# joyecnu/STTODE

Measured on AMD Instinct MI355X. Metric: predicted-trajectories/sec (20-sample best-of-K), higher is better.
Workload: dtype f32

## Files before the change

sttode_amd/csrc/chain32.hip:

```cpp
#include "chain.hpp"
#include "latency_bodies.hpp"
#include "frontend_body.hpp"
#include "api_util.hpp"
#include "../../include/sttode_hip.h"
#include <cstdlib>
#include <cstddef>

#ifdef C32_DIAG_TRACE
__shared__ long long g_tr_ph[4];
#define C32_TRACE_BEGIN() long long _tr_t0 = 0, _tr_c0 = 0; if (threadIdx.x == 0 && A.dbg) { _tr_t0 = __builtin_amdgcn_s_memrealtime(); _tr_c0 = __builtin_amdgcn_s_memtime(); }
#define C32_TRACE_END(kind) do { if (threadIdx.x == 0 && A.dbg) { \
        const long long _t1 = __builtin_amdgcn_s_memrealtime(); unsigned _hw, _xcc; \
        asm volatile("s_getreg_b32 %0, hwreg(HW_REG_HW_ID)" : "=s"(_hw)); asm volatile("s_getreg_b32 %0, hwreg(HW_REG_XCC_ID)" : "=s"(_xcc)); \
        const unsigned long long _r = atomicAdd((unsigned long long*)A.dbg, 1ull); if ((long long)_r >= A.dbg[1]) break;  \
        long long* _p = A.dbg + 8 + _r * 12; _p[0] = A.trace_tag; _p[1] = blockIdx.x; _p[2] = (kind); _p[3] = _tr_t0; _p[4] = _t1; _p[5] = _hw; _p[6] = _xcc; \
        _p[8] = g_tr_ph[0]; _p[9] = g_tr_ph[1]; _p[10] = g_tr_ph[2]; _p[7] = __builtin_amdgcn_s_memtime() - _tr_c0; _p[11] = g_tr_ph[3]; } } while (0)
#define C32_TRACE_PHASE(i) do { if (threadIdx.x == 0) g_tr_ph[i] = __builtin_amdgcn_s_memrealtime(); } while (0)
#else
#define C32_TRACE_PHASE(i) do { } while (0)
#define C32_TRACE_BEGIN() do { } while (0)
#define C32_TRACE_END(kind) do { } while (0)
#endif

#include "role_body.hpp"

typedef float f32x16 __attribute__((ext_vector_type(16)));

#ifdef C32_DIAG_NOGATES
#define C32_SIG(x) ((x) * 1e-3f)
#define C32_TANH(x) ((x) * 1e-3f)
#else
#define C32_SIG(x) sigmoid_prescaled(x)
#define C32_TANH(x) tanh_prescaled(x)
#endif

#define C32_TILE 256
#define C32_CMAX 3
#define C32_RING (2 * C32_CMAX * C32_TILE)
#define C32_SLOT 256

struct Role32Args {
    const f32x4* pool; const int2* prog; int prog_len; const float* consts;
    const float* enc_in; const int* last;
    const float* g_in; const float* attn; int ld_attn;
    const float* xpad; int ldx;
    float* pf; float* state0; float* A0x; float* A0y; float* A1y;
    int n, Tp, kte, nwg;
    float ode_time;
    int prio;
    int* counter;
    float* zgen; unsigned zkey0, zkey1; int K;
    const float* past; const int* scene_ptr; int S; float* scene_orig; int* agent_scene;
    float* enc_in_w; float* xpad_w; float* cur_w; float* orig_w; int* last_w;
    float* m_ade; float* m_fde;
};

struct ChainArgs {
    const float* A0x; const float* A0y; const float* A1y;
    const f32x4* pool;
    const int2* prog; int prog_len;
    const float* consts;
    const float* z;
    const float* xpad; int ldx;
    const float* cur; const float* orig;
    float* pred;
    float* park;
    int* counter;
    int ncols, K, Tp, Tf2;
    int persistent;
    const float* m_gt; float* m_ade; float* m_fde; float m_scale;
    int nworkers;
    long long* dbg;
    int trace_tag;
    int xcd_map;
    RoleArgs R;
    Role32Args R32;
};

template <int NY> struct C32Const {
    static constexpr int b2x = 0, b3x = 256, b2y = 288, b3y = 544, gb = 544 + 32 * NY, cb = gb + 384, b2m = cb + 32,
                         b3m = b2m + 256, total = b3m + 32 * NY;
};

__device__ __forceinline__ f32x16 splat16(float v) {
    f32x16 r;
#pragma unroll
    for (int e = 0; e < 16; ++e) r[e] = v;
    return r;
}
__device__ __forceinline__ f32x16 relu16(f32x16 v) {
#pragma unroll
    for (int e = 0; e < 16; ++e) v[e] = fmaxf(v[e], 0.f);
    return v;
}
__device__ __forceinline__ f32x16 ldrows(const float* p, int h) {
    f32x16 r;
#pragma unroll
    for (int a = 0; a < 4; ++a) {
        const f32x4 v = ld4(p + 8 * a + 4 * h);
        r[4 * a + 0] = v[0]; r[4 * a + 1] = v[1]; r[4 * a + 2] = v[2]; r[4 * a + 3] = v[3];
    }
    return r;
}

typedef const __attribute__((address_space(4))) int KProg;

template <int BUF, bool GEN, bool DYN = false>
struct ChainStreamT {
    static constexpr int kBuf = BUF;
    static constexpr int kPieces = (BUF / 64 + 3) / 4, kPairs = (kPieces + 1) / 2;
    const char* pool; KProg* prog; f32x4* ring;
    unsigned ring_addr, loff;
    unsigned qoff, qend;
    int par, lane, wave;
    int2 ld_v, ld_w;
    bool fetched;
    int cnt;
    const char* nsrc[kPairs]; unsigned nm0[kPairs]; int ncnt, npc;
#ifdef C32_DIAG_STAMPS
    long long t_bar, gap_cyc, gap_n, gap_cal;
#endif
    __device__ __forceinline__ int2 entry_at(unsigned off) const {
        const KProg* e = reinterpret_cast<const KProg*>(reinterpret_cast<const __attribute__((address_space(4))) char*>(prog) + off);
        return make_int2(e[0], e[1]);
    }
    __device__ __forceinline__ unsigned next_off(unsigned off) const { return off + 8 >= qend ? 0u : off + 8; }
    __device__ __forceinline__ void stage(int2 ev, int buf) {
        ncnt = __builtin_amdgcn_readfirstlane(ev.y);
        npc = GEN ? (ncnt - wave + 3) >> 2 : ncnt;
        const size_t src = (size_t)(unsigned)__builtin_amdgcn_readfirstlane(ev.x) * (GEN ? 16u : C32_TILE * 16u) + (unsigned)wave * 1024u;
        const unsigned dst = __builtin_amdgcn_readfirstlane(ring_addr + (unsigned)buf * (BUF * 16) + (unsigned)wave * 1024u);
#pragma unroll
        for (int k = 0; k < kPairs; ++k) {
            nsrc[k] = pool + (src + 4096u * (2 * k + 1));
            nm0[k] = dst + 4096u * (2 * k + 1);
            asm volatile("" : "+s"(nsrc[k]), "+s"(nm0[k]));
        }
        asm volatile("" : "+s"(npc));
    }
    __device__ __forceinline__ void issue(int N) {
#ifndef C32_DIAG_NODMA
#pragma unroll
        for (int k = 0; k < kPairs; ++k) {
            if (N > 0 ? 2 * k < N : 2 * k < npc) {
                glds16_sv<-4096>(nsrc[k], loff, nm0[k] - 4096u);
                if (2 * k + 1 < kPieces && (N > 0 ? 2 * k + 1 < N : 2 * k + 1 < npc)) glds16_m0<0>(nsrc[k], loff);
            }
        }
#endif
    }
    __device__ __forceinline__ void init(const f32x4* pool_, const int2* prog_, int len_, f32x4* ring_) {
        pool = reinterpret_cast<const char*>(pool_); prog = (KProg*)prog_; ring = ring_;
        ring_addr = __builtin_amdgcn_readfirstlane(lds_addr(ring_));
        lane = threadIdx.x & 63;
        loff = (unsigned)lane * 16;
        wave = __builtin_amdgcn_readfirstlane(threadIdx.x >> 6);
        par = 0;
        qend = (unsigned)len_ * 8u;
        const int2 e0 = entry_at(0);
        stage(e0, 0);
        issue(0);
        cnt = e0.y;
        qoff = next_off(0);
        stage(entry_at(qoff), 1);
        qoff = next_off(qoff);
        fetched = false;
#ifdef C32_DIAG_STAMPS
        gap_cyc = 0; gap_n = 0;
        const long long c0 = __builtin_amdgcn_s_memtime();
        asm volatile("s_waitcnt lgkmcnt(0)" ::: "memory");
        gap_cal = __builtin_amdgcn_s_memtime() - c0;
        t_bar = 0;
#endif
    }
    __device__ __forceinline__ void fetch() { ld_v = entry_at(qoff); qoff = next_off(qoff); fetched = true; }
    __device__ __forceinline__ void fetch_more() { ld_w = entry_at(qoff); qoff = next_off(qoff); }
    __device__ __forceinline__ void take_prefetched() { ld_v = ld_w; fetched = true; }
    __device__ __forceinline__ void stamp_gap() {
#ifdef C32_DIAG_STAMPS
        asm volatile("s_waitcnt lgkmcnt(0)" ::: "memory");
        const long long c1 = __builtin_amdgcn_s_memtime();
        asm volatile("s_waitcnt lgkmcnt(0)" ::: "memory");
        if (t_bar) { gap_cyc += c1 - t_bar; ++gap_n; }
#endif
    }
    __device__ __forceinline__ void begin(int N = 0) {
        __builtin_amdgcn_sched_barrier(0);
#ifdef C32_DIAG_CHECK
        if (!GEN && N > 0 && ncnt != N) __builtin_trap();
#endif
        cnt = ncnt;
        issue(GEN || DYN ? 0 : N);
        stamp_gap();
        __builtin_amdgcn_sched_barrier(0);
    }
    __device__ __forceinline__ const f32x4* cur() const { return ring + par * BUF + lane; }
    __device__ __forceinline__ void end(bool has_entry = false) {
        __builtin_amdgcn_sched_barrier(0);
#ifdef C32_DIAG_CHECK
        if (has_entry && !fetched) __builtin_trap();
#endif
        if (!has_entry && !fetched) fetch();
        stage(ld_v, par);
        __builtin_amdgcn_sched_barrier(0);
#ifndef C32_DIAG_NOBARRIER
        asm volatile("s_waitcnt vmcnt(0)" ::: "memory");
        __syncthreads();
#endif
#ifdef C32_DIAG_STAMPS
        t_bar = __builtin_amdgcn_s_memtime();
        asm volatile("s_waitcnt lgkmcnt(0)" ::: "memory");
#endif
        par ^= 1;
        fetched = false;
        __builtin_amdgcn_sched_barrier(0);
    }
};
typedef ChainStreamT<C32_CMAX * C32_TILE, false> ChainStream;

__device__ __forceinline__ void tile_mma(f32x16& acc, const f32x4* __restrict__ t, const f32x16& B) {
#pragma unroll
    for (int g = 0; g < 4; ++g) {
        const f32x4 a = t[g * 64];
#pragma unroll
        for (int r = 0; r < 4; ++r) acc = __builtin_amdgcn_mfma_f32_32x32x2f32(a[r], B[4 * g + r], acc, 0, 0, 0);
    }
}

__device__ __forceinline__ void gather_rows(const void* base, unsigned voff, unsigned slot_addr) {
    glds16_sv<0>(base, voff, slot_addr);
    glds16_sv<32>(base, voff, slot_addr + 1024);
    glds16_sv<64>(base, voff, slot_addr + 2048);
    glds16_sv<96>(base, voff, slot_addr + 3072);
}
__device__ __forceinline__ unsigned row_off(int row, int width, int h) { return (unsigned)row * (unsigned)(width * 4) + (unsigned)h * 16; }

struct Frag { f32x4 a[4]; };
__device__ __forceinline__ void ldfrag(Frag& f, const f32x4* __restrict__ t) {
#pragma unroll
    for (int g = 0; g < 4; ++g) f.a[g] = t[g * 64];
}
__device__ __forceinline__ void tile_mma2(f32x16& acc, const Frag& cur, const f32x16& B, Frag& nxt, const f32x4* __restrict__ tn) {
#pragma unroll
    for (int g = 0; g < 4; ++g) {
        if (g == 2 && tn) {
            ldfrag(nxt, tn);
            __builtin_amdgcn_sched_barrier(0);
        }
#pragma unroll
        for (int r = 0; r < 4; ++r) acc = __builtin_amdgcn_mfma_f32_32x32x2f32(cur.a[g][r], B[4 * g + r], acc, 0, 0, 0);
    }
}

template <class ST>
__device__ __forceinline__ void tile_mma2f(ST& st, f32x16& acc, const Frag& cur, const f32x16& B, Frag& nxt, const f32x4* __restrict__ tn, int nf = 1) {
#pragma unroll
    for (int g = 0; g < 4; ++g) {
        if (g == 2) {
            __builtin_amdgcn_sched_barrier(0);
            if (nf >= 1) st.fetch();
            if (nf >= 2) st.fetch_more();
            if (tn) ldfrag(nxt, tn);
            __builtin_amdgcn_sched_barrier(0);
        }
#pragma unroll
        for (int r = 0; r < 4; ++r) acc = __builtin_amdgcn_mfma_f32_32x32x2f32(cur.a[g][r], B[4 * g + r], acc, 0, 0, 0);
    }
}

template <int KH, class ST>
__device__ __forceinline__ void mlp_l12(ST& st, const f32x4* slot, const f32x4* zslot, const f32x16* Bh, const float* tab, unsigned aoff,
                                        const float* tab_next, unsigned aoff_next, f32x16 (&acc2)[8], int lane) {
    const unsigned slot_addr = __builtin_amdgcn_readfirstlane(lds_addr(slot));
    constexpr int KT1 = 1 + KH;
    static_assert((KT1 + 8) % 3 == 0, "hidden tile must be a whole number of chunks");
#pragma unroll
    for (int R = 0; R < 8; ++R) acc2[R] = splat16(0.f);
#pragma unroll 1
    for (int ht = 0; ht < 16; ++ht) {
        f32x16 h1, zb;
#pragma unroll
        for (int a = 0; a < 4; ++a) {
            const f32x4 v = slot[a * 64 + lane];
            h1[4 * a + 0] = v[0]; h1[4 * a + 1] = v[1]; h1[4 * a + 2] = v[2]; h1[4 * a + 3] = v[3];
        }
#pragma unroll
        for (int a = 0; a < 4; ++a) {
            const f32x4 v = zslot[a * 64 + lane];
            zb[4 * a + 0] = v[0]; zb[4 * a + 1] = v[1]; zb[4 * a + 2] = v[2]; zb[4 * a + 3] = v[3];
        }
        asm volatile("s_waitcnt lgkmcnt(0)" ::: "memory");
        __builtin_amdgcn_sched_barrier(0);
        const bool nl = ht + 1 < 16;
        const void* nb = nl ? (const void*)(reinterpret_cast<const char*>(tab) + 128 * (ht + 1)) : (const void*)tab_next;
        const unsigned no = nl ? aoff : aoff_next;
        Frag fr[2];
#pragma unroll
        for (int i = 0; i < KT1 + 8; ++i) {
            if (i % 3 == 0) {
                if (i > 0) st.end();
                ldfrag(fr[i & 1], st.cur());
                st.begin(3);
                if (i == 0) {
#ifndef C32_DIAG_NOGATHER
                    gather_rows(nb, no, slot_addr);
#endif
                    __builtin_amdgcn_sched_barrier(0);
                }
            }
            const f32x4* tn = (i % 3 < 2) ? st.cur() + (i % 3 + 1) * C32_TILE : nullptr;
            if (i == 0) {
                tile_mma2f(st, h1, fr[i & 1], zb, fr[(i + 1) & 1], tn);
            } else if (i < KT1) {
                if (i % 3 == 0) tile_mma2f(st, h1, fr[i & 1], Bh[i - 1], fr[(i + 1) & 1], tn);
                else tile_mma2(h1, fr[i & 1], Bh[i - 1], fr[(i + 1) & 1], tn);
            } else {
                if (i == KT1) h1 = relu16(h1);
                if (i % 3 == 0) tile_mma2f(st, acc2[i - KT1], fr[i & 1], h1, fr[(i + 1) & 1], tn);
                else tile_mma2(acc2[i - KT1], fr[i & 1], h1, fr[(i + 1) & 1], tn);
            }
        }
        st.end();
    }
}

template <int NO, int NEXT = 0, class ST>
__device__ __forceinline__ void mlp_l3(ST& st, f32x16 (&acc2)[8], const float* __restrict__ b2, const float* __restrict__ b3,
                                       f32x16 (&out)[NO], int h) {
#pragma unroll
    for (int R = 0; R < 8; ++R) {
        STT_FENCE();
        const f32x16 b = ldrows(b2 + 32 * R, h);
        acc2[R] = relu16(acc2[R] + b);
        asm volatile("" : "+v"(acc2[R]));
    }
    STT_FENCE();
#pragma unroll
    for (int o = 0; o < NO; ++o) out[o] = ldrows(b3 + 32 * o, h);
    Frag fr[2];
#pragma unroll
    for (int i = 0; i < 8 * NO; ++i) {
        if (i % 3 == 0) {
            if (i > 0) st.end();
            ldfrag(fr[i & 1], st.cur());
            const int left = 8 * NO - (i + 3);
            st.begin(left >= 3 ? 3 : left > 0 ? left : NEXT);
        }
        const f32x4* tn = (i % 3 < 2 && i + 1 < 8 * NO) ? st.cur() + (i % 3 + 1) * C32_TILE : nullptr;
        if (i % 3 == 0) tile_mma2f(st, out[i / 8], fr[i & 1], acc2[i % 8], fr[(i + 1) & 1], tn);
        else tile_mma2(out[i / 8], fr[i & 1], acc2[i % 8], fr[(i + 1) & 1], tn);
    }
    st.end();
}

typedef __bf16 bf16x8 __attribute__((ext_vector_type(8)));
typedef __bf16 bf16x2 __attribute__((ext_vector_type(2)));
typedef float f32x2v __attribute__((ext_vector_type(2)));
typedef unsigned u32x4v __attribute__((ext_vector_type(4)));
#define C32_TILE_B3 384
#define C32_BUF_B3 (C32_CMAX * C32_TILE_B3)
struct B3 { bf16x8 p[3][2]; };
__device__ __forceinline__ float bf_lo(unsigned u) { return __uint_as_float(u << 16); }
__device__ __forceinline__ float bf_hi(unsigned u) { return __uint_as_float(u & 0xffff0000u); }
__device__ __forceinline__ void split3(const f32x16& x, B3& o) {
#pragma unroll
    for (int kb = 0; kb < 2; ++kb) {
        unsigned hi[4], mi[4], lo[4];
#pragma unroll
        for (int q = 0; q < 4; ++q) {
            const float x0 = x[8 * kb + 2 * q], x1 = x[8 * kb + 2 * q + 1];
            const f32x2v v = {x0, x1};
            hi[q] = __builtin_bit_cast(unsigned, __builtin_convertvector(v, bf16x2));
            const float r0 = x0 - bf_lo(hi[q]), r1 = x1 - bf_hi(hi[q]);
            const f32x2v rv = {r0, r1};
            mi[q] = __builtin_bit_cast(unsigned, __builtin_convertvector(rv, bf16x2));
            const f32x2v qv = {r0 - bf_lo(mi[q]), r1 - bf_hi(mi[q])};
            lo[q] = __builtin_bit_cast(unsigned, __builtin_convertvector(qv, bf16x2));
        }
        const u32x4v H = {hi[0], hi[1], hi[2], hi[3]}, M = {mi[0], mi[1], mi[2], mi[3]}, L = {lo[0], lo[1], lo[2], lo[3]};
        o.p[0][kb] = __builtin_bit_cast(bf16x8, H);
        o.p[1][kb] = __builtin_bit_cast(bf16x8, M);
        o.p[2][kb] = __builtin_bit_cast(bf16x8, L);
    }
}
struct Frag6 { f32x4 a[6]; };
__device__ __forceinline__ void ldfrag6(Frag6& f, const f32x4* __restrict__ t) {
#pragma unroll
    for (int i = 0; i < 6; ++i) f.a[i] = t[i * 64];
}
__device__ __forceinline__ void tile_mma_b3(f32x16& acc, const Frag6& cur, const B3& B, Frag6& nxt, const f32x4* __restrict__ tn) {
#pragma unroll
    for (int kb = 0; kb < 2; ++kb) {
        if (kb == 1 && tn) {
            ldfrag6(nxt, tn);
            __builtin_amdgcn_sched_barrier(0);
        }
        const bf16x8 ah = __builtin_bit_cast(bf16x8, cur.a[kb * 3 + 0]), am = __builtin_bit_cast(bf16x8, cur.a[kb * 3 + 1]),
                     al = __builtin_bit_cast(bf16x8, cur.a[kb * 3 + 2]);
        acc = __builtin_amdgcn_mfma_f32_32x32x16_bf16(al, B.p[0][kb], acc, 0, 0, 0);
        acc = __builtin_amdgcn_mfma_f32_32x32x16_bf16(ah, B.p[2][kb], acc, 0, 0, 0);
        acc = __builtin_amdgcn_mfma_f32_32x32x16_bf16(am, B.p[1][kb], acc, 0, 0, 0);
        acc = __builtin_amdgcn_mfma_f32_32x32x16_bf16(am, B.p[0][kb], acc, 0, 0, 0);
        acc = __builtin_amdgcn_mfma_f32_32x32x16_bf16(ah, B.p[1][kb], acc, 0, 0, 0);
        acc = __builtin_amdgcn_mfma_f32_32x32x16_bf16(ah, B.p[0][kb], acc, 0, 0, 0);
    }
}
__device__ __forceinline__ void tile_mma_b3n(f32x16& acc, const f32x4* __restrict__ t, const B3& B) {
    Frag6 f, dummy;
    ldfrag6(f, t);
    tile_mma_b3(acc, f, B, dummy, nullptr);
}
template <int KH, bool PRE, class ST>
__device__ __forceinline__ void mlp_l12_b3(ST& st, const f32x4* slot, const f32x4* zslot, const f32x16* Bh, const float* tab, unsigned aoff,
                                           const float* tab_next, unsigned aoff_next, f32x16 (&acc2)[8], int lane) {
    const unsigned slot_addr = __builtin_amdgcn_readfirstlane(lds_addr(slot));
    constexpr int KT1 = 1 + KH;
    static_assert((KT1 + 8) % 3 == 0, "hidden tile must be a whole number of chunks");
#pragma unroll
    for (int R = 0; R < 8; ++R) acc2[R] = splat16(0.f);
    B3 Bz;
    if (KH == 0) {
        f32x16 zb;
#pragma unroll
        for (int a = 0; a < 4; ++a) {
            const f32x4 v = zslot[a * 64 + lane];
            zb[4 * a + 0] = v[0]; zb[4 * a + 1] = v[1]; zb[4 * a + 2] = v[2]; zb[4 * a + 3] = v[3];
        }
        split3(zb, Bz);
    }
#pragma unroll 1
    for (int ht = 0; ht < 16; ++ht) {
        f32x16 h1;
// ... 159 lines not shown
}

template <bool ZS, class ST>
__device__ __forceinline__ f32x16 gru32_conv(ST& st, const float* cb, const f32x16& d, int t, int Tp, int h, bool pre) {
    f32x16 e = ldrows(cb, h);
    Frag fa, fb;
    if (ZS) {
        const int k0 = 2 * t - 2, k1 = 2 * t + 3;
        const int g0 = (k0 > 0 ? k0 : 0) >> 3, g1 = (k1 < 2 * Tp - 1 ? k1 : 2 * Tp - 1) >> 3;
        const f32x4* tc = st.cur();
#pragma unroll
        for (int g = 0; g < 4; ++g)
            if (g >= g0 && g <= g1) fa.a[g] = tc[g * 64];
        st.begin(3);
#pragma unroll
        for (int g = 0; g < 4; ++g)
            if (g >= g0 && g <= g1)
#pragma unroll
                for (int r = 0; r < 4; ++r) e = __builtin_amdgcn_mfma_f32_32x32x2f32(fa.a[g][r], d[4 * g + r], e, 0, 0, 0);
        __builtin_amdgcn_sched_barrier(0);
        if (pre) st.take_prefetched();
        else st.fetch();
    } else {
        ldfrag(fa, st.cur());
        st.begin(3);
        tile_mma2f(st, e, fa, d, fb, nullptr, pre ? 0 : 1);
        if (pre) st.take_prefetched();
    }
    e = relu16(e);
    st.end();
    return e;
}

template <bool ZS, class ST>
__device__ __forceinline__ void gru32_steps(ST& st, const float* gb, const float* cb, const f32x16& d, f32x16 (&hs)[3], int Tp, int h) {
    if (ZS) {
        const f32x16 e = gru32_conv<ZS>(st, cb, d, 0, Tp, h, false);
        Frag fa, fb;
#pragma unroll
        for (int j = 0; j < 3; ++j) {
            STT_FENCE();
            f32x16 ar = ldrows(gb + 0 * 96 + 32 * j, h);
            ldfrag(fa, st.cur()); st.begin(3);
            tile_mma2f(st, ar, fa, e, fb, nullptr);
            st.end(); ldfrag(fa, st.cur() + 1 * C32_TILE); st.begin(3);
#pragma unroll
            for (int r = 0; r < 16; ++r) ar[r] = C32_SIG(ar[r]);
            STT_FENCE();
            f32x16 az = ldrows(gb + 1 * 96 + 32 * j, h);
            tile_mma2f(st, az, fa, e, fb, nullptr, 2);
            st.end(); st.begin(3);
            st.take_prefetched();
#pragma unroll
            for (int r = 0; r < 16; ++r) az[r] = C32_SIG(az[r]);
            STT_FENCE();
            f32x16 an = ldrows(gb + 3 * 96 + 32 * j, h);
            {
                const f32x16 bi = ldrows(gb + 2 * 96 + 32 * j, h);
#pragma unroll
                for (int r = 0; r < 16; ++r) an[r] = fmaf(ar[r], an[r], bi[r]);
            }
            st.end(); ldfrag(fa, st.cur() + 2 * C32_TILE);
            if (j < 2) st.begin(3); else st.begin();
            STT_FENCE();
            tile_mma2f(st, an, fa, e, fb, nullptr, (j == 2 && 1 < Tp) ? 2 : 1);
            st.end();
#pragma unroll
            for (int r = 0; r < 16; ++r) {
                const float ng = C32_TANH(an[r]);
                hs[j][r] = fmaf(az[r], 0.f - ng, ng);
            }
        }
    }
#pragma unroll 1
    for (int t = ZS ? 1 : 0; t < Tp; ++t) {
        const f32x16 e = gru32_conv<ZS>(st, cb, d, t, Tp, h, ZS);
        Frag fa, fb;
        f32x16 hn[3];
#pragma unroll
        for (int j = 0; j < 3; ++j) {
            STT_FENCE();
            f32x16 ar = ldrows(gb + 0 * 96 + 32 * j, h);
            ldfrag(fa, st.cur()); st.begin(3);
            tile_mma2f(st, ar, fa, e, fb, st.cur() + 1 * C32_TILE);
            tile_mma2(ar, fb, hs[0], fa, st.cur() + 2 * C32_TILE);
            tile_mma2(ar, fa, hs[1], fb, nullptr);
            st.end(); ldfrag(fa, st.cur()); st.begin(3);
            tile_mma2f(st, ar, fa, hs[2], fb, st.cur() + 1 * C32_TILE);
#pragma unroll
            for (int r = 0; r < 16; ++r) ar[r] = C32_SIG(ar[r]);
            STT_FENCE();
            f32x16 az = ldrows(gb + 1 * 96 + 32 * j, h);
            tile_mma2(az, fb, e, fa, st.cur() + 2 * C32_TILE);
            tile_mma2(az, fa, hs[0], fb, nullptr);
            st.end(); ldfrag(fa, st.cur()); st.begin(3);
            tile_mma2f(st, az, fa, hs[1], fb, st.cur() + 1 * C32_TILE);
            tile_mma2(az, fb, hs[2], fa, st.cur() + 2 * C32_TILE);
#pragma unroll
            for (int r = 0; r < 16; ++r) az[r] = C32_SIG(az[r]);
            STT_FENCE();
            f32x16 an = ldrows(gb + 3 * 96 + 32 * j, h);
            tile_mma2(an, fa, hs[0], fb, nullptr);
            st.end(); ldfrag(fa, st.cur());
            if (j < 2) st.begin(3); else st.begin();
            tile_mma2f(st, an, fa, hs[1], fb, st.cur() + 1 * C32_TILE, (ZS && j == 2 && t + 1 < Tp) ? 2 : 1);
            tile_mma2(an, fb, hs[2], fa, st.cur() + 2 * C32_TILE);
            {
                const f32x16 bi = ldrows(gb + 2 * 96 + 32 * j, h);
#pragma unroll
                for (int r = 0; r < 16; ++r) an[r] = fmaf(ar[r], an[r], bi[r]);
            }
            STT_FENCE();
            tile_mma2(an, fa, e, fb, nullptr);
            st.end();
#pragma unroll
            for (int r = 0; r < 16; ++r) {
                const float ng = C32_TANH(an[r]);
                hn[j][r] = fmaf(az[r], hs[j][r] - ng, ng);
            }
        }
#pragma unroll
        for (int j = 0; j < 3; ++j) hs[j] = hn[j];
    }

}

#include "role32.hpp"

__device__ __forceinline__ int opaque(int v) { asm volatile("" : "+v"(v)); return v; }

#ifdef C32_DIAG_STAMPS
#define C32_STAMP(k) do { if (threadIdx.x == 0 && A.dbg && gi < 4) { A.dbg[((size_t)blockIdx.x * 4 + gi) * 16 + 2 * (k)] = __builtin_amdgcn_s_memtime(); \
                                                                    A.dbg[((size_t)blockIdx.x * 4 + gi) * 16 + 2 * (k) + 1] = __builtin_amdgcn_s_memrealtime(); } } while (0)
#else
#define C32_STAMP(k) do { } while (0)
#endif

__host__ __device__ __forceinline__ int fused_block_of(long b, long T, long G, long K, long lead) {
    auto roles_upto = [&](long x) { const long c = (8 * (x + lead + 1) + K - 1) / K; return c < T ? c : T; };
    long lo = -1, hi = G - 1;
    while (lo < hi) {
        const long mid = (lo + hi + 1) >> 1;
        if (mid + roles_upto(mid) <= b) lo = mid; else hi = mid - 1;
    }
    if (lo >= 0 && lo + roles_upto(lo) == b) return (int)lo;
    return -1 - (int)(b - (lo + 1));
}

__host__ __device__ __forceinline__ int xcd_group(int b, int G) {
    const int x = b & 7, i = b >> 3, q = G >> 3, r = G & 7;
    return x * q + (x < r ? x : r) + i;
}

template <int NY, int FUSE, bool B3M, bool ZS>
__global__ __launch_bounds__(256, 2) void traj_chain_kernel(ChainArgs A) {
    constexpr bool kDynCount = !B3M && ((NY == 1 && FUSE == 2 && !ZS) || (NY == 2 && FUSE == 1 && ZS));
    typedef ChainStreamT<B3M ? C32_BUF_B3 : C32_CMAX * C32_TILE, B3M, kDynCount> Stream;
    extern __shared__ __attribute__((aligned(16))) char smem[];
    f32x4* ring = reinterpret_cast<f32x4*>(smem);
    f32x4* slots = ring + 2 * Stream::kBuf;
    f32x4* zslots = slots + 4 * C32_SLOT;
    float* cst = reinterpret_cast<float*>(zslots + 4 * C32_SLOT);
    int* sq = reinterpret_cast<int*>(cst + C32Const<NY>::total);
    typedef C32Const<NY> CO;

    const int lane = threadIdx.x & 63, c = lane & 31, h = lane >> 5;
    const int wave = __builtin_amdgcn_readfirstlane(threadIdx.x >> 6);
    const f32x4* slot = slots + wave * C32_SLOT;
    const f32x4* zslot = zslots + wave * C32_SLOT;
    const unsigned slot_addr = __builtin_amdgcn_readfirstlane(lds_addr(slot));
    const unsigned zslot_addr = __builtin_amdgcn_readfirstlane(lds_addr(zslot));
    const int ngroups = (A.ncols + 127) >> 7;

    C32_TRACE_BEGIN();
    if (FUSE == 2 && (int)blockIdx.x < A.R32.nwg) {
        role32_body<ZS>(*(KRole32Args*)((const __attribute__((address_space(4))) char*)__builtin_amdgcn_kernarg_segment_ptr() + offsetof(ChainArgs, R32)),
                    blockIdx.x, smem);
        C32_TRACE_END(1);
        return;
    }
    if (FUSE == 1 && A.R.split && (int)blockIdx.x < 5 * A.R.ntiles) {
        split_role(A.R, (A.ncols + A.K - 1) / A.K, A.Tp, A.ldx, A.xpad, blockIdx.x, smem);
        C32_TRACE_END(1);
        return;
    }
    int fb = FUSE == 0 ? (int)blockIdx.x : FUSE == 2 ? (int)blockIdx.x - A.R32.nwg : A.R.split ? (int)blockIdx.x - 5 * A.R.ntiles
                                                : fused_block_of(blockIdx.x, A.R.ntiles, ngroups, A.K, A.R.lead);
    if (FUSE && A.xcd_map && fb >= 0) fb = xcd_group(fb, ngroups);
    if (FUSE == 1 && fb < 0) {
        agent_role(A.R, (A.ncols + A.K - 1) / A.K, A.Tp, A.ldx, A.xpad, -1 - fb, smem);
        C32_TRACE_END(1);
        return;
    }
    for (int i = threadIdx.x; i < CO::total; i += blockDim.x) cst[i] = A.consts[i];
    if (threadIdx.x == 0) sq[0] = FUSE == 2 ? fb : (FUSE == 0 && A.persistent) ? atomicAdd(A.counter, 1) : FUSE ? fb : (int)blockIdx.x;
    if (FUSE == 1) {
        const int g0 = fb;
        const int c_lo = g0 * 128, c_hi = (c_lo + 127 < A.ncols ? c_lo + 127 : A.ncols - 1);
        const int t_lo = (c_lo / A.K) >> 4, t_hi = (c_hi / A.K) >> 4;
        if (wave == 0) {
            const bool ok = A.R.split ? wait_tiles(A.R.pflags, 3 * t_lo, 3 * t_hi + 2, A.R.flags + A.R.ntiles, lane, A.R.tmo_host)
                                      : wait_tiles(A.R.flags, t_lo, t_hi, A.R.flags + A.R.ntiles, lane, A.R.tmo_host);
            if (!ok && lane == 0) sq[0] = -1;
        }
    }
    __syncthreads();
    C32_TRACE_PHASE(3);
    int g = sq[0];
    if (FUSE == 1 && g < 0) {
        for (int i = threadIdx.x; i < 128 * A.Tf2; i += blockDim.x) {
            const size_t o = (size_t)fb * 128 * A.Tf2 + i;
            if (o < (size_t)A.ncols * A.Tf2) A.pred[o] = __builtin_nanf("");
        }
        return;
    }
    if (g >= ngroups) return;
    Stream st;
    st.init(A.pool, A.prog, A.prog_len, ring);

    auto col_of = [&](int gg) { int col = gg * 128 + wave * 32 + c; return col < A.ncols ? col : A.ncols - 1; };
    {
        const int c0 = col_of(g);
        gather_rows(A.A0x, row_off(c0 / A.K, 512, h), slot_addr);
        gather_rows(A.z, row_off(c0, 32, h), zslot_addr);
    }
    asm volatile("s_waitcnt vmcnt(0)" ::: "memory");
    __syncthreads();

    int gi = 0;
    (void)gi;
    while (true) {
        C32_STAMP(0);
        const int col = g * 128 + wave * 32 + c;
        int colc = col < A.ncols ? col : A.ncols - 1;
        int agent = colc / A.K;
        const bool live = col < A.ncols;
        __syncthreads();
        if (threadIdx.x == 0)
            sq[1] = (FUSE == 2 && A.persistent && ngroups > A.nworkers) ? A.nworkers + atomicAdd(A.counter, 1)
                    : (FUSE == 0 && A.persistent) ? atomicAdd(A.counter, 1) : ngroups;
// ... 138 lines not shown
                        atomicMin(reinterpret_cast<unsigned*>(A.m_ade) + agent, __float_as_uint(adev));
                        atomicMin(reinterpret_cast<unsigned*>(A.m_fde) + agent, __float_as_uint(fdl));
                    }
                }
            }
        }
        C32_STAMP(4);
#ifdef C32_DIAG_STAMPS
        if (threadIdx.x == 0 && A.dbg && gi < 4) {
            long long* o = A.dbg + ((size_t)blockIdx.x * 4 + gi) * 16 + 10;
            o[0] = st.gap_cyc; o[1] = st.gap_n; o[2] = st.gap_cal;
        }
        st.gap_cyc = 0; st.gap_n = 0;
#endif
        ++gi;
        g = gnext;
        if (g >= ngroups) break;
    }
    C32_TRACE_END(0);
}

struct Gru32Args {
    const float* xin; int ldx;
    const f32x4* pool; const int2* prog; int prog_len;
    const float* consts;
    float* state;
    int ncols, Tp;
};
template <bool ZS>
__global__ __launch_bounds__(256, 2) void gru32_kernel(Gru32Args A) {
    extern __shared__ __attribute__((aligned(16))) char smem[];
    f32x4* ring = reinterpret_cast<f32x4*>(smem);
    float* cst = reinterpret_cast<float*>(ring + C32_RING);
    const int lane = threadIdx.x & 63, c = lane & 31, h = lane >> 5;
    const int wave = __builtin_amdgcn_readfirstlane(threadIdx.x >> 6);
    for (int i = threadIdx.x; i < 416; i += blockDim.x) cst[i] = A.consts[i];
    __syncthreads();
    ChainStream st;
    st.init(A.pool, A.prog, A.prog_len, ring);
    const int col = blockIdx.x * 128 + wave * 32 + c;
    const int colc = col < A.ncols ? col : A.ncols - 1;
    f32x16 d;
    {
        const float* xp = A.xin + (size_t)colc * A.ldx;
#pragma unroll
        for (int a = 0; a < 4; ++a) {
            f32x4 v = splat4(0.f);
            if (8 * a + 4 * h < A.ldx) v = ld4(xp + 8 * a + 4 * h);
#pragma unroll
            for (int b = 0; b < 4; ++b) d[4 * a + b] = v[b];
        }
    }
    asm volatile("s_waitcnt vmcnt(0)" ::: "memory");
    __syncthreads();
    f32x16 hs[3];
#pragma unroll
    for (int j = 0; j < 3; ++j) hs[j] = splat16(0.f);
    gru32_steps<ZS>(st, cst, cst + 384, d, hs, A.Tp, h);
    if (col < A.ncols) {
#pragma unroll
        for (int j = 0; j < 3; ++j)
#pragma unroll
            for (int a = 0; a < 4; ++a) {
                const f32x4 v = {hs[j][4 * a], hs[j][4 * a + 1], hs[j][4 * a + 2], hs[j][4 * a + 3]};
                st4(A.state + (size_t)col * 96 + 32 * j + 8 * a + 4 * h, v);
            }
    }
}

static int chain_cus() {
    static int n = 0;
    if (!n) {
        int dev = 0;
        hipDeviceProp_t p;
        if (hipGetDevice(&dev) == hipSuccess && hipGetDeviceProperties(&p, dev) == hipSuccess) n = p.multiProcessorCount;
        if (n <= 0) n = 256;
    }
    return n;
}
static int gru_zero_skip() {
    static const int v = getenv("STTODE_GRU_ZERO_SKIP") ? atoi(getenv("STTODE_GRU_ZERO_SKIP")) != 0 : 1;
    return v;
}
static int chain_lds(int NY, bool b3 = false) { return ((b3 ? 2 * C32_BUF_B3 : C32_RING) + 8 * C32_SLOT) * 16 + (1216 + 64 * NY) * 4 + 16; }

static int role_lds(int Tp) {
    const int e = (Tp * 256 + 512) * 16, g = (2 * 6 * 64 + 2 * 24 * 64 + 2 * 4 * 64) * 16;
    return e > g ? e : g;
}

static int role32_lds() { return C32_RING * 16 + R32C::total * 4; }

template <int NY, int FUSE, bool B3M = false> static int chain_launch(ChainArgs a, int wgs_per_cu, hipStream_t s) {
    void (*kern)(ChainArgs) = gru_zero_skip() ? traj_chain_kernel<NY, FUSE, B3M, true> : traj_chain_kernel<NY, FUSE, B3M, false>;
    STT_SET_LDS_ONCE(kern, 96 * 1024);
    const int ngroups = (a.ncols + 127) / 128;
    int grid = ngroups;
    if (FUSE == 1) grid = (a.R.split ? 5 : 1) * a.R.ntiles + ngroups;
    else if (FUSE == 2) {
        int workers = ngroups;
        if (a.persistent && workers > 2 * chain_cus()) workers = 2 * chain_cus();
        grid = a.R32.nwg + (a.ncols > 0 ? workers : 0);
        a.nworkers = workers;
        if (workers < ngroups) a.xcd_map = 0;
    }
    int lds = chain_lds(NY, B3M);
    if (FUSE == 1 && lds < role_lds(a.Tp)) lds = role_lds(a.Tp);
    if (FUSE == 2 && a.R32.nwg > 0 && lds < role32_lds()) lds = role32_lds();
    if (wgs_per_cu == 1 && lds < 84 * 1024) lds = 84 * 1024;
    STT_REQUIRE(lds <= 96 * 1024, "sttode_traj_chain: dynamic LDS beyond the 96 KiB the kernel is registered for");
    STT_REQUIRE((long)a.ncols * 128 <= 0xffffffffL && (long)((a.ncols + a.K - 1) / a.K) * 2048 <= 0xffffffffL,
                "sttode_traj_chain: z / per-agent table rows beyond the 32-bit byte offsets of the gathers");
    if (FUSE == 1) STT_HIP(hipMemsetAsync(a.R.flags, 0, (((size_t)(a.R.split ? 5 : 1) * a.R.ntiles + 1) * 4 + 15) / 16 * 16, s));
    hipLaunchKernelGGL(kern, dim3(grid), dim3(256), lds, s, a);
    STT_HIP(hipGetLastError());
    return 0;
}

extern "C" int sttode_gru_cols32(const float* xin, int ldx, const float* pool, const int* prog, int prog_len, const float* consts,
                                 float* state, int ncols, int Tp, void* stream) {
    STT_REQUIRE(xin && pool && prog && consts && state, "sttode_gru_cols32: null pointer");
    STT_REQUIRE(ncols > 0 && Tp >= 1 && (ldx == 16 || ldx == 32) && 2 * Tp <= ldx, "sttode_gru_cols32: bad ncols/Tp/ldx");
    STT_REQUIRE(prog_len == 13 * Tp, "sttode_gru_cols32: chunk program must hold 13 entries per step");
    Gru32Args a;
    a.xin = xin; a.ldx = ldx; a.pool = (const f32x4*)pool; a.prog = (const int2*)prog; a.prog_len = prog_len; a.consts = consts;
    a.state = state; a.ncols = ncols; a.Tp = Tp;
    const int lds = C32_RING * 16 + 416 * 4;
    hipLaunchKernelGGL(gru_zero_skip() ? gru32_kernel<true> : gru32_kernel<false>, dim3((ncols + 127) / 128), dim3(256), lds, (hipStream_t)stream, a);
    STT_HIP(hipGetLastError());
    return 0;
}

__global__ __launch_bounds__(256, 2) void sampler_qnet32_kernel(QNet32Args Q) {
    extern __shared__ __attribute__((aligned(16))) char smem[];
    f32x4* ring = reinterpret_cast<f32x4*>(smem);
    const int lane = threadIdx.x & 63, c = lane & 31, h = lane >> 5;
    const int wave = __builtin_amdgcn_readfirstlane(threadIdx.x >> 6);
    ChainStream st;
    st.init(Q.pool, Q.prog, Q.prog_len, ring);
    const int col = blockIdx.x * 128 + wave * 32 + c;
    const bool live = col < Q.n;
    const int colc = live ? col : Q.n - 1;
    f32x16 P[4];
#pragma unroll
    for (int kt = 0; kt < 4; ++kt) P[kt] = ldrows(Q.pf + (size_t)colc * 128 + 32 * kt, h);
    asm volatile("s_waitcnt vmcnt(0)" ::: "memory");
    __syncthreads();
    TileFeed<ChainStream> fd(st);
    fd.open();
    qnet32(fd, Q, P, col, colc, live, h);
    fd.close();
}

static long sampler_tiles(const SttodeSamplerPlan* p) {
    const long h1t = p->h1 / 32, h2t = p->h2 / 32;
    return 8 + h1t * (2 + h2t) + (long)p->K * h2t * (p->eps_mode ? 2 : 1);
}
const char* stt_sampler_plan_check(const SttodeSamplerPlan* p, int K) {
    if (!p || !p->pool || !p->prog || !p->biases) return "sampler plan: null pool / program / biases";
    if (p->nz != 32) return "sampler plan: nz must be 32 (one MFMA tile of rows per sample)";
    if (p->K <= 0 || (K > 0 && p->K != K)) return "sampler plan: K must be positive and equal the model's sample_k";
    if (p->h1 <= 0 || p->h1 % 32 || p->h2 <= 0 || p->h2 % 32 || p->h2 > 256) return "sampler plan: hidden widths must be multiples of 32, h2 <= 256";
    if (p->eps_mode < 0 || p->eps_mode > 2 || (p->eps_mode != 0 && !p->eps)) return "sampler plan: eps_mode 0 (mean) | 1 (shared [nz]) | 2 (per agent [n][nz]); eps required unless 0";
    if (p->prog_len <= 0 || p->prog_len > 4096) return "sampler plan: prog_len must be in [1, 4096]";
    if (3L * p->prog_len < sampler_tiles(p)) return "sampler plan: chunk program too short for the widths (<= 3 tiles per chunk)";
    return nullptr;
}
// ... 204 lines not shown
```

Before: 86.76 million.

## Prefetch first fragment group of next chunk into private LDS before barrier

Adds an 'early' streaming mode in which each wave DMAs the first fragment group of the next weight chunk into a private LDS region behind the ring. The last tile of a chunk reads it before the block barrier and issues the next tile's first MFMAs, so the barrier wait overlaps with matrix work. The MLP, output and GRU gate loops are restructured to use this, and kDynCount is extended to NY=2 fused zero-skip. The cost is 4 KiB more LDS per workgroup and more complex scheduling that could reduce occupancy or break the alignment of the prefetched rows.

```diff
diff --git a/sttode_amd/csrc/chain32.hip b/sttode_amd/csrc/chain32.hip
--- a/sttode_amd/csrc/chain32.hip
+++ b/sttode_amd/csrc/chain32.hip
@@ -105,9 +105,13 @@
 
 typedef const __attribute__((address_space(4))) int KProg;
 
-template <int BUF, bool GEN, bool DYN = false>
+template <int BUF, bool GEN, bool DYN = false, int PRIV = 0>
 struct ChainStreamT {
+    static constexpr bool EARLY = PRIV > 0;
+    static_assert(!(EARLY && GEN), "the private first group is a piece of a PK32 tile");
+    static_assert(!EARLY || PRIV >= 2 * BUF, "the private slots lie behind the ring");
     static constexpr int kBuf = BUF;
+    static constexpr bool kEarly = EARLY;
     static constexpr int kPieces = (BUF / 64 + 3) / 4, kPairs = (kPieces + 1) / 2;
     const char* pool; KProg* prog; f32x4* ring;
     unsigned ring_addr, loff;
@@ -176,6 +180,12 @@
     __device__ __forceinline__ void fetch() { ld_v = entry_at(qoff); qoff = next_off(qoff); fetched = true; }
     __device__ __forceinline__ void fetch_more() { ld_w = entry_at(qoff); qoff = next_off(qoff); }
     __device__ __forceinline__ void take_prefetched() { ld_v = ld_w; fetched = true; }
+    __device__ __forceinline__ void first_group() {
+#ifndef C32_DIAG_NODMA
+        const unsigned back = 4096u + (unsigned)wave * 1024u;
+        glds16_sv<0>(nsrc[0] - back, loff, ring_addr + PRIV * 16 + (unsigned)wave * 1024u);
+#endif
+    }
     __device__ __forceinline__ void stamp_gap() {
 #ifdef C32_DIAG_STAMPS
         asm volatile("s_waitcnt lgkmcnt(0)" ::: "memory");
@@ -205,6 +215,22 @@
         __builtin_amdgcn_sched_barrier(0);
 #ifndef C32_DIAG_NOBARRIER
         asm volatile("s_waitcnt vmcnt(0)" ::: "memory");
+#endif
+        end_arrive();
+    }
+    __device__ __forceinline__ f32x4 end_read() {
+#ifdef C32_DIAG_CHECK
+        if (!fetched) __builtin_trap();
+#endif
+        stage(ld_v, par);
+#ifndef C32_DIAG_NOBARRIER
+        asm volatile("s_waitcnt vmcnt(0)" ::: "memory");
+#endif
+        return ring[PRIV + wave * 64 + lane];
+    }
+    __device__ __forceinline__ void end_arrive() {
+        __builtin_amdgcn_sched_barrier(0);
+#ifndef C32_DIAG_NOBARRIER
         __syncthreads();
 #endif
 #ifdef C32_DIAG_STAMPS
@@ -253,14 +279,59 @@
 }
 
 template <class ST>
-__device__ __forceinline__ void tile_mma2f(ST& st, f32x16& acc, const Frag& cur, const f32x16& B, Frag& nxt, const f32x4* __restrict__ tn, int nf = 1) {
+__device__ __forceinline__ void tile_mma2f(ST& st, f32x16& acc, const Frag& cur, const f32x16& B, Frag& nxt, const f32x4* __restrict__ tn, int nf = 1,
+                                           bool fg = false) {
 #pragma unroll
     for (int g = 0; g < 4; ++g) {
         if (g == 2) {
             __builtin_amdgcn_sched_barrier(0);
             if (nf >= 1) st.fetch();
             if (nf >= 2) st.fetch_more();
+            if (fg) st.first_group();
             if (tn) ldfrag(nxt, tn);
+            __builtin_amdgcn_sched_barrier(0);
+        }
+#pragma unroll
+        for (int r = 0; r < 4; ++r) acc = __builtin_amdgcn_mfma_f32_32x32x2f32(cur.a[g][r], B[4 * g + r], acc, 0, 0, 0);
+    }
+}
+
+template <class ST>
+__device__ __forceinline__ void tile_last_e(ST& st, f32x16& acc, const Frag& cur, const f32x16& B, Frag& nxt, f32x16& accN, const f32x16& BN) {
+#pragma unroll
+    for (int g = 0; g < 4; ++g) {
+        if (g == 2) {
+            __builtin_amdgcn_sched_barrier(0);
+            nxt.a[0] = st.end_read();
+            __builtin_amdgcn_sched_barrier(0);
+        }
+#pragma unroll
+        for (int r = 0; r < 4; ++r) acc = __builtin_amdgcn_mfma_f32_32x32x2f32(cur.a[g][r], B[4 * g + r], acc, 0, 0, 0);
+    }
+#pragma unroll
+    for (int r = 0; r < 4; ++r) accN = __builtin_amdgcn_mfma_f32_32x32x2f32(nxt.a[0][r], BN[r], accN, 0, 0, 0);
+    st.end_arrive();
+}
+template <class ST>
+__device__ __forceinline__ void ldfrag_rest(const ST& st, Frag& f, Frag& second, bool two) {
+    const f32x4* __restrict__ t = st.cur();
+#pragma unroll
+    for (int g = 1; g < 4; ++g) f.a[g] = t[g * 64];
+    if (two) second.a[0] = t[C32_TILE];
+}
+template <class ST>
+__device__ __forceinline__ void tile_first_e(ST& st, f32x16& acc, const Frag& cur, const f32x16& B, Frag& nxt, const f32x4* __restrict__ tn, int nf, bool fg) {
+#pragma unroll
+    for (int g = 1; g < 4; ++g) {
+        if (g == 2) {
+            __builtin_amdgcn_sched_barrier(0);
+            if (nf >= 1) st.fetch();
+            if (nf >= 2) st.fetch_more();
+            if (fg) st.first_group();
+            if (tn) {
+#pragma unroll
+                for (int k = 1; k < 4; ++k) nxt.a[k] = tn[k * 64];
+            }
             __builtin_amdgcn_sched_barrier(0);
         }
 #pragma unroll
@@ -295,11 +366,19 @@
         const void* nb = nl ? (const void*)(reinterpret_cast<const char*>(tab) + 128 * (ht + 1)) : (const void*)tab_next;
         const unsigned no = nl ? aoff : aoff_next;
         Frag fr[2];
+        constexpr bool E = ST::kEarly;
+        static_assert(!E || KT1 % 3 == 1, "the relu must not fall on a chunk boundary, nor on the tile in front of one");
 #pragma unroll
         for (int i = 0; i < KT1 + 8; ++i) {
+            const bool pre = E && i % 3 == 0 && i > 0;
+            const bool ee = E && i - i % 3 + 3 < KT1 + 8;
             if (i % 3 == 0) {
-                if (i > 0) st.end();
-                ldfrag(fr[i & 1], st.cur());
+                if (pre) {
+                    ldfrag_rest(st, fr[i & 1], fr[(i + 1) & 1], true);
+                } else {
+                    if (i > 0) st.end();
+                    ldfrag(fr[i & 1], st.cur());
+                }
                 st.begin(3);
                 if (i == 0) {
 #ifndef C32_DIAG_NOGATHER
@@ -310,13 +389,17 @@
             }
             const f32x4* tn = (i % 3 < 2) ? st.cur() + (i % 3 + 1) * C32_TILE : nullptr;
             if (i == 0) {
-                tile_mma2f(st, h1, fr[i & 1], zb, fr[(i + 1) & 1], tn);
+                tile_mma2f(st, h1, fr[i & 1], zb, fr[(i + 1) & 1], tn, 1, ee);
             } else if (i < KT1) {
-                if (i % 3 == 0) tile_mma2f(st, h1, fr[i & 1], Bh[i - 1], fr[(i + 1) & 1], tn);
+                if (pre) tile_first_e(st, h1, fr[i & 1], Bh[i - 1], fr[(i + 1) & 1], tn, 1, ee);
+                else if (i % 3 == 0) tile_mma2f(st, h1, fr[i & 1], Bh[i - 1], fr[(i + 1) & 1], tn);
+                else if (ee && i % 3 == 2) tile_last_e(st, h1, fr[i & 1], Bh[i - 1], fr[(i + 1) & 1], h1, Bh[i]);
                 else tile_mma2(h1, fr[i & 1], Bh[i - 1], fr[(i + 1) & 1], tn);
             } else {
                 if (i == KT1) h1 = relu16(h1);
-                if (i % 3 == 0) tile_mma2f(st, acc2[i - KT1], fr[i & 1], h1, fr[(i + 1) & 1], tn);
+                if (pre) tile_first_e(st, acc2[i - KT1], fr[i & 1], h1, fr[(i + 1) & 1], tn, 1, ee);
+                else if (i % 3 == 0) tile_mma2f(st, acc2[i - KT1], fr[i & 1], h1, fr[(i + 1) & 1], tn);
+                else if (ee && i % 3 == 2) tile_last_e(st, acc2[i - KT1], fr[i & 1], h1, fr[(i + 1) & 1], acc2[i + 1 - KT1], h1);
                 else tile_mma2(acc2[i - KT1], fr[i & 1], h1, fr[(i + 1) & 1], tn);
             }
         }
@@ -338,16 +421,25 @@
 #pragma unroll
     for (int o = 0; o < NO; ++o) out[o] = ldrows(b3 + 32 * o, h);
     Frag fr[2];
+    constexpr bool E = ST::kEarly;
 #pragma unroll
     for (int i = 0; i < 8 * NO; ++i) {
+        const bool pre = E && i % 3 == 0 && i > 0;
+        const bool ee = E && i - i % 3 + 3 < 8 * NO;
         if (i % 3 == 0) {
-            if (i > 0) st.end();
-            ldfrag(fr[i & 1], st.cur());
+            if (pre) {
+                ldfrag_rest(st, fr[i & 1], fr[(i + 1) & 1], i + 1 < 8 * NO);
+            } else {
+                if (i > 0) st.end();
+                ldfrag(fr[i & 1], st.cur());
+            }
             const int left = 8 * NO - (i + 3);
             st.begin(left >= 3 ? 3 : left > 0 ? left : NEXT);
         }
         const f32x4* tn = (i % 3 < 2 && i + 1 < 8 * NO) ? st.cur() + (i % 3 + 1) * C32_TILE : nullptr;
-        if (i % 3 == 0) tile_mma2f(st, out[i / 8], fr[i & 1], acc2[i % 8], fr[(i + 1) & 1], tn);
+        if (pre) tile_first_e(st, out[i / 8], fr[i & 1], acc2[i % 8], fr[(i + 1) & 1], tn, 1, ee);
+        else if (i % 3 == 0) tile_mma2f(st, out[i / 8], fr[i & 1], acc2[i % 8], fr[(i + 1) & 1], tn, 1, ee);
+        else if (ee && i % 3 == 2) tile_last_e(st, out[i / 8], fr[i & 1], acc2[i % 8], fr[(i + 1) & 1], out[(i + 1) / 8], acc2[(i + 1) % 8]);
         else tile_mma2(out[i / 8], fr[i & 1], acc2[i % 8], fr[(i + 1) & 1], tn);
     }
     st.end();
@@ -673,6 +765,46 @@
             STT_FENCE();
             f32x16 ar = ldrows(gb + 0 * 96 + 32 * j, h);
             ldfrag(fa, st.cur()); st.begin(3);
+            if (ST::kEarly) {
+                const int nf = (ZS && j == 2 && t + 1 < Tp) ? 2 : 1;
+                tile_mma2f(st, ar, fa, e, fb, st.cur() + 1 * C32_TILE, 1, true);
+                tile_mma2(ar, fb, hs[0], fa, st.cur() + 2 * C32_TILE);
+                tile_last_e(st, ar, fa, hs[1], fb, ar, hs[2]);
+                ldfrag_rest(st, fb, fa, true); st.begin(3);
+                tile_first_e(st, ar, fb, hs[2], fa, st.cur() + 1 * C32_TILE, 1, true);
+#pragma unroll
+                for (int r = 0; r < 16; ++r) ar[r] = C32_SIG(ar[r]);
+                STT_FENCE();
+                f32x16 az = ldrows(gb + 1 * 96 + 32 * j, h);
+                tile_mma2(az, fa, e, fb, st.cur() + 2 * C32_TILE);
+                tile_last_e(st, az, fb, hs[0], fa, az, hs[1]);
+                ldfrag_rest(st, fa, fb, true); st.begin(3);
+                tile_first_e(st, az, fa, hs[1], fb, st.cur() + 1 * C32_TILE, 1, true);
+                tile_mma2(az, fb, hs[2], fa, st.cur() + 2 * C32_TILE);
+#pragma unroll
+                for (int r = 0; r < 16; ++r) az[r] = C32_SIG(az[r]);
+                STT_FENCE();
+                f32x16 an = ldrows(gb + 3 * 96 + 32 * j, h);
+                tile_last_e(st, an, fa, hs[0], fb, an, hs[1]);
+                ldfrag_rest(st, fb, fa, true);
+                if (j < 2) st.begin(3); else st.begin();
+                tile_first_e(st, an, fb, hs[1], fa, st.cur() + 1 * C32_TILE, nf, false);
+                tile_mma2(an, fa, hs[2], fb, st.cur() + 2 * C32_TILE);
+                {
+                    const f32x16 bi = ldrows(gb + 2 * 96 + 32 * j, h);
+#pragma unroll
+                    for (int r = 0; r < 16; ++r) an[r] = fmaf(ar[r], an[r], bi[r]);
+                }
+                STT_FENCE();
+                tile_mma2(an, fb, e, fa, nullptr);
+                st.end();
+#pragma unroll
+                for (int r = 0; r < 16; ++r) {
+                    const float ng = C32_TANH(an[r]);
+                    hn[j][r] = fmaf(az[r], hs[j][r] - ng, ng);
+                }
+                continue;
+            }
             tile_mma2f(st, ar, fa, e, fb, st.cur() + 1 * C32_TILE);
             tile_mma2(ar, fb, hs[0], fa, st.cur() + 2 * C32_TILE);
             tile_mma2(ar, fa, hs[1], fb, nullptr);
@@ -745,8 +877,10 @@
 
 template <int NY, int FUSE, bool B3M, bool ZS>
 __global__ __launch_bounds__(256, 2) void traj_chain_kernel(ChainArgs A) {
-    constexpr bool kDynCount = !B3M && ((NY == 1 && FUSE == 2 && !ZS) || (NY == 2 && FUSE == 1 && ZS));
-    typedef ChainStreamT<B3M ? C32_BUF_B3 : C32_CMAX * C32_TILE, B3M, kDynCount> Stream;
+    constexpr bool kDynCount = !B3M && ((NY == 1 && FUSE == 2 && !ZS) || (NY == 2 && FUSE == 1 && ZS) || (NY == 2 && FUSE == 2 && ZS));
+    constexpr bool kEarly = !B3M && !kDynCount && NY < 3;
+    constexpr int kPriv = kEarly ? C32_RING + 8 * C32_SLOT + (C32Const<NY>::total * 4 + 16) / 16 : 0;
+    typedef ChainStreamT<B3M ? C32_BUF_B3 : C32_CMAX * C32_TILE, B3M, kDynCount, kPriv> Stream;
     extern __shared__ __attribute__((aligned(16))) char smem[];
     f32x4* ring = reinterpret_cast<f32x4*>(smem);
     f32x4* slots = ring + 2 * Stream::kBuf;
@@ -1051,7 +1185,9 @@
     static const int v = getenv("STTODE_GRU_ZERO_SKIP") ? atoi(getenv("STTODE_GRU_ZERO_SKIP")) != 0 : 1;
     return v;
 }
-static int chain_lds(int NY, bool b3 = false) { return ((b3 ? 2 * C32_BUF_B3 : C32_RING) + 8 * C32_SLOT) * 16 + (1216 + 64 * NY) * 4 + 16; }
+static int chain_lds(int NY, bool b3 = false) {
+    return ((b3 ? 2 * C32_BUF_B3 : C32_RING) + 8 * C32_SLOT) * 16 + (1216 + 64 * NY) * 4 + 16 + (b3 ? 0 : 4 * 1024);
+}
 
 static int role_lds(int Tp) {
     const int e = (Tp * 256 + 512) * 16, g = (2 * 6 * 64 + 2 * 24 * 64 + 2 * 4 * 64) * 16;
```

Result: no change. 86.67 million (-0.1%).
